# KwonGihyun/TweedieMix

Hardware: AMD Instinct MI355X
Metric: denoise steps/sec @ SDXL 1024^2 K=3 concepts (fusion phase); images/sec at 1/2/4/8 GPUs (higher is better)
Workload: dtype bf16

## Files before the change

### tweediemix_amd/csrc/conv_io.hip

```cpp
#include "common.h"

namespace {

struct PreMap { float w[16]; float b[4]; int on; };

template <int CIN>
__global__ void __launch_bounds__(256) conv_in_kernel(const float* __restrict__ x, const float* __restrict__ w,
                                                      const float* __restrict__ bias, bf16_t* __restrict__ y,
                                                      int B, int H, int W, int Cout, const PreMap pm) {
    extern __shared__ __attribute__((aligned(16))) float s_w[];
    constexpr int KK = 9 * CIN;
    const int tid = threadIdx.x, lane = tid & 63;
    const int q = __builtin_amdgcn_readfirstlane(tid >> 6);
    for (int i = tid; i < Cout * KK / 4; i += 256) ((float4*)s_w)[i] = ((const float4*)w)[i];
    __syncthreads();
    const int64_t npix = (int64_t)B * H * W;
    for (int64_t tile = blockIdx.x; tile * 64 < npix; tile += gridDim.x) {
    int64_t pix = tile * 64 + lane;
    const bool live = pix < npix;
    if (!live) pix = npix - 1;
    const int b = (int)(pix / ((int64_t)H * W)); const int rem = (int)(pix - (int64_t)b * H * W);
    const int oy = rem / W, ox = rem - oy * W;
    float patch[KK];
#pragma unroll
    for (int ky = 0; ky < 3; ++ky)
#pragma unroll
        for (int kx = 0; kx < 3; ++kx) {
            const int iy = oy + ky - 1, ix = ox + kx - 1;
            const bool ok = iy >= 0 && iy < H && ix >= 0 && ix < W;
            float v[CIN];
#pragma unroll
            for (int ci = 0; ci < CIN; ++ci) v[ci] = ok ? x[(((int64_t)b * CIN + ci) * H + iy) * W + ix] : 0.f;
            if (pm.on && CIN == 4) {
                float u[4];
#pragma unroll
                for (int co = 0; co < 4; ++co)
                    u[co] = ok ? pm.b[co] + pm.w[co * 4 + 0] * v[0] + pm.w[co * 4 + 1] * v[1] + pm.w[co * 4 + 2] * v[2] + pm.w[co * 4 + 3] * v[3] : 0.f;
#pragma unroll
                for (int co = 0; co < 4; ++co) v[co] = u[co];
            }
#pragma unroll
            for (int ci = 0; ci < CIN; ++ci) patch[(ky * 3 + kx) * CIN + ci] = v[ci];
        }
    const int cpq = Cout / 4;
    for (int c0 = q * cpq; c0 < (q + 1) * cpq; c0 += 8) {
        float o[8];
#pragma unroll 2
        for (int j = 0; j < 8; ++j) {
            const float* wr = s_w + (c0 + j) * KK;
            float a = bias ? bias[c0 + j] : 0.f;
#pragma unroll
            for (int k = 0; k < KK; ++k) a += patch[k] * wr[k];
            o[j] = a;
        }
        if (live) *(uint4*)(y + pix * Cout + c0) = pack8(o);
    }
    }
}

template <int CIN>
int launch_conv_in(unsigned nb, int smem, hipStream_t st, const float* x, const float* w, const float* bias, bf16_t* y, int B, int H, int W, int Cout, const PreMap& pm) {
    static int attr_smem = 0;
    if (smem > 64 * 1024 && smem > attr_smem) {
        hipError_t e = hipFuncSetAttribute((const void*)conv_in_kernel<CIN>, hipFuncAttributeMaxDynamicSharedMemorySize, smem);
        if (e != hipSuccess) TMIX_FAIL((int)e, "hipFuncSetAttribute: %s", hipGetErrorString(e));
        attr_smem = smem;
    }
    conv_in_kernel<CIN><<<nb, 256, smem, st>>>(x, w, bias, y, B, H, W, Cout, pm);
    TMIX_LAUNCH_CHECK();
    return TMIX_OK;
}

__global__ void __launch_bounds__(256) conv_out_kernel(const bf16_t* __restrict__ x, const bf16_t* __restrict__ w,
                                                       const float* __restrict__ bias, float* __restrict__ y,
                                                       int B, int H, int W, int Cin, int Cout) {
    const int lane = threadIdx.x & 63, fr = lane & 15, fg = lane >> 4;
    const int64_t npix = (int64_t)B * H * W;
    const int64_t pbase = ((int64_t)blockIdx.x * 4 + (threadIdx.x >> 6)) * 16;
    if (pbase >= npix) return;
    int64_t pix = pbase + fr; if (pix > npix - 1) pix = npix - 1;
    const int b = (int)(pix / ((int64_t)H * W)); const int rem = (int)(pix - (int64_t)b * H * W);
    const int oy = rem / W, ox = rem - oy * W;
    const int co = fr < Cout ? fr : Cout - 1;
    const bf16_t* wrow = w + (int64_t)co * 9 * Cin;
    f32x4 acc = {0.f, 0.f, 0.f, 0.f};
    const frag_ab zero = {0, 0, 0, 0, 0, 0, 0, 0};
    for (int tap = 0; tap < 9; ++tap) {
        const int ky = tap / 3, kx = tap - ky * 3;
        const int iy = oy + ky - 1, ix = ox + kx - 1;
        const bool ok = iy >= 0 && iy < H && ix >= 0 && ix < W;
        const bf16_t* src = x + (((int64_t)b * H + (ok ? iy : 0)) * W + (ok ? ix : 0)) * Cin;
        for (int c = 0; c < Cin; c += 32) {
            frag_ab a = *(const frag_ab*)(src + c + fg * 8);
            if (!ok) a = zero;
            const frag_ab wf = *(const frag_ab*)(wrow + tap * Cin + c + fg * 8);
            acc = __builtin_amdgcn_mfma_f32_16x16x32_bf16(a, wf, acc, 0, 0, 0);
        }
    }
    if (fr < Cout) {
        const float bv = bias ? bias[fr] : 0.f;
#pragma unroll
        for (int r = 0; r < 4; ++r) {
            const int64_t pp = pbase + fg * 4 + r;
            if (pp < npix) {
                const int bb = (int)(pp / ((int64_t)H * W)); const int64_t rr = pp - (int64_t)bb * H * W;
                y[((int64_t)bb * Cout + fr) * H * W + rr] = acc[r] + bv;
            }
        }
    }
}

}

extern "C" int tmix_conv_in(const float* x_nchw, const float* w_ohwi, const float* bias, void* y_nhwc,
                            int B, int Cin, int H, int W, int Cout, void* stream) {
    return tmix_conv_in_pre(x_nchw, w_ohwi, bias, y_nhwc, B, Cin, H, W, Cout, nullptr, nullptr, stream);
}

extern "C" int tmix_conv_in_pre(const float* x_nchw, const float* w_ohwi, const float* bias, void* y_nhwc,
                                int B, int Cin, int H, int W, int Cout, const float* pre_w, const float* pre_b, void* stream) {
    if (!x_nchw || !w_ohwi || !y_nhwc) TMIX_FAIL(TMIX_EINVAL, "conv_in: null pointer");
    if (B <= 0 || H <= 0 || W <= 0 || Cout <= 0) TMIX_FAIL(TMIX_ESHAPE, "conv_in: bad shape");
    if (!aligned16(y_nhwc)) TMIX_FAIL(TMIX_EALIGN, "conv_in: output must be 16-byte aligned");
    if (Cout % 32) TMIX_FAIL(TMIX_ESHAPE, "conv_in: Cout=%d must be a multiple of 32", Cout);
    if (Cin != 3 && Cin != 4 && Cin != 8) TMIX_FAIL(TMIX_ESHAPE, "conv_in: Cin=%d (3: RGB image, 4: image latent, 8: video latent + image-latent features)", Cin);
    if (Cin != 4 && pre_w) TMIX_FAIL(TMIX_EINVAL, "conv_in: the latent pre-map is defined for 4 channels");
    if ((Cout * 9 * Cin) % 4) TMIX_FAIL(TMIX_ESHAPE, "conv_in: Cout*9*Cin must be a multiple of 4");
    if (!aligned16(w_ohwi)) TMIX_FAIL(TMIX_EALIGN, "conv_in: weights must be 16-byte aligned");
    const int64_t npix = (int64_t)B * H * W;
    const int64_t ntiles = (npix + 63) / 64;
    const int smem = Cout * 9 * Cin * 4;
    const int per_cu = smem > 80 * 1024 ? 1 : (smem > 52 * 1024 ? 2 : 3);
    const unsigned nb = (unsigned)(ntiles < 256 * per_cu ? ntiles : 256 * per_cu);
    if (smem > 150 * 1024) TMIX_FAIL(TMIX_ESHAPE, "conv_in: Cout=%d too large for the LDS weight stage", Cout);
    PreMap pm = {};
    if (pre_w) {
        pm.on = 1;
        for (int i = 0; i < 16; ++i) pm.w[i] = pre_w[i];
        for (int i = 0; i < 4; ++i) pm.b[i] = pre_b ? pre_b[i] : 0.f;
    }
    hipStream_t st = (hipStream_t)stream;
    bf16_t* y = (bf16_t*)y_nhwc;
    switch (Cin) {
        case 8:  return launch_conv_in<8>(nb, smem, st, x_nchw, w_ohwi, bias, y, B, H, W, Cout, pm);
        case 3:  return launch_conv_in<3>(nb, smem, st, x_nchw, w_ohwi, bias, y, B, H, W, Cout, pm);
        default: return launch_conv_in<4>(nb, smem, st, x_nchw, w_ohwi, bias, y, B, H, W, Cout, pm);
    }
}

extern "C" int tmix_conv_out(const void* x_nhwc, const void* w_ohwi, const float* bias, float* y_nchw,
                             int B, int Cin, int H, int W, int Cout, void* stream) {
    if (!x_nhwc || !w_ohwi || !y_nchw) TMIX_FAIL(TMIX_EINVAL, "conv_out: null pointer");
    if (B <= 0 || H <= 0 || W <= 0 || Cout <= 0 || Cout > 16 || (Cin % 32)) TMIX_FAIL(TMIX_ESHAPE, "conv_out: Cin=%d (%%32) Cout=%d (<=16)", Cin, Cout);
    if (!aligned16(x_nhwc) || !aligned16(w_ohwi)) TMIX_FAIL(TMIX_EALIGN, "conv_out: pointers must be 16-byte aligned");
    const int64_t npix = (int64_t)B * H * W;
    const unsigned nb = (unsigned)((npix + 63) / 64);
    conv_out_kernel<<<nb, 256, 0, (hipStream_t)stream>>>((const bf16_t*)x_nhwc, (const bf16_t*)w_ohwi, bias, y_nchw, B, H, W, Cin, Cout);
    TMIX_LAUNCH_CHECK();
    return TMIX_OK;
}
```

Baseline: 32.96.

## Tile conv_out through LDS with halo reuse and widen conv_in blocks

conv_out now stages a (TH+2)x18 halo tile of the NHWC input and all filter rows into padded LDS, then runs MFMA over 2D spatial tiles with unrolled channel chunks. This replaces per-lane global loads that re-read each input pixel nine times. conv_in moves to 512-thread blocks covering 128 pixels with two pixels' worth of waves, and packs outputs pairwise. It also switches to explicit fma and deliberately unfused mul-add for the tail taps and pre-map rows, apparently to match reference rounding. The costs are higher LDS use per block, which may reduce occupancy, and extra staging work per block.

```diff
diff --git a/tweediemix_amd/csrc/conv_io.hip b/tweediemix_amd/csrc/conv_io.hip
--- a/tweediemix_amd/csrc/conv_io.hip
+++ b/tweediemix_amd/csrc/conv_io.hip
@@ -4,19 +4,26 @@
 
 struct PreMap { float w[16]; float b[4]; int on; };
 
+constexpr int CONV_IN_SPLIT = 12;
+__device__ __forceinline__ float mul_add_rounded(float a, float p, float w) {
+#pragma clang fp contract(off)
+    const float t = p * w;
+    return a + t;
+}
+
 template <int CIN>
-__global__ void __launch_bounds__(256) conv_in_kernel(const float* __restrict__ x, const float* __restrict__ w,
+__global__ void __launch_bounds__(512) conv_in_kernel(const float* __restrict__ x, const float* __restrict__ w,
                                                       const float* __restrict__ bias, bf16_t* __restrict__ y,
                                                       int B, int H, int W, int Cout, const PreMap pm) {
     extern __shared__ __attribute__((aligned(16))) float s_w[];
     constexpr int KK = 9 * CIN;
     const int tid = threadIdx.x, lane = tid & 63;
-    const int q = __builtin_amdgcn_readfirstlane(tid >> 6);
-    for (int i = tid; i < Cout * KK / 4; i += 256) ((float4*)s_w)[i] = ((const float4*)w)[i];
+    const int wv = __builtin_amdgcn_readfirstlane(tid >> 6), q = wv & 3, half = wv >> 2;
+    for (int i = tid; i < Cout * KK / 4; i += 512) ((float4*)s_w)[i] = ((const float4*)w)[i];
     __syncthreads();
     const int64_t npix = (int64_t)B * H * W;
-    for (int64_t tile = blockIdx.x; tile * 64 < npix; tile += gridDim.x) {
-    int64_t pix = tile * 64 + lane;
+    for (int64_t tile = blockIdx.x; tile * 128 < npix; tile += gridDim.x) {
+    int64_t pix = tile * 128 + half * 64 + lane;
     const bool live = pix < npix;
     if (!live) pix = npix - 1;
     const int b = (int)(pix / ((int64_t)H * W)); const int rem = (int)(pix - (int64_t)b * H * W);
@@ -34,8 +41,13 @@
             if (pm.on && CIN == 4) {
                 float u[4];
 #pragma unroll
-                for (int co = 0; co < 4; ++co)
-                    u[co] = ok ? pm.b[co] + pm.w[co * 4 + 0] * v[0] + pm.w[co * 4 + 1] * v[1] + pm.w[co * 4 + 2] * v[2] + pm.w[co * 4 + 3] * v[3] : 0.f;
+                for (int co = 0; co < 4; ++co) {
+                    float t = pm.b[co];
+#pragma unroll
+                    for (int ci = 0; ci < 4; ++ci)
+                        t = co < 2 ? __builtin_fmaf(pm.w[co * 4 + ci], v[ci], t) : mul_add_rounded(t, pm.w[co * 4 + ci], v[ci]);
+                    u[co] = ok ? t : 0.f;
+                }
 #pragma unroll
                 for (int co = 0; co < 4; ++co) v[co] = u[co];
             }
@@ -44,16 +56,25 @@
         }
     const int cpq = Cout / 4;
     for (int c0 = q * cpq; c0 < (q + 1) * cpq; c0 += 8) {
-        float o[8];
-#pragma unroll 2
-        for (int j = 0; j < 8; ++j) {
-            const float* wr = s_w + (c0 + j) * KK;
-            float a = bias ? bias[c0 + j] : 0.f;
-#pragma unroll
-            for (int k = 0; k < KK; ++k) a += patch[k] * wr[k];
-            o[j] = a;
-        }
-        if (live) *(uint4*)(y + pix * Cout + c0) = pack8(o);
+        uint32_t ow[4] = {0, 0, 0, 0};
+#pragma unroll 1
+        for (int jp = 0; jp < 4; ++jp) {
+            float o[2];
+#pragma unroll
+            for (int j = 0; j < 2; ++j) {
+                const float* wr = s_w + (c0 + 2 * jp + j) * KK;
+                float a = bias ? bias[c0 + 2 * jp + j] : 0.f;
+#pragma unroll
+                for (int k = 0; k < KK - CONV_IN_SPLIT; ++k) a = __builtin_fmaf(patch[k], wr[k], a);
+#pragma unroll
+                for (int k = KK - CONV_IN_SPLIT; k < KK; ++k) a = mul_add_rounded(a, patch[k], wr[k]);
+                o[j] = a;
+            }
+            const uint32_t pk = pack_bf2(o[0], o[1]);
+#pragma unroll
+            for (int t = 0; t < 4; ++t) ow[t] = jp == t ? pk : ow[t];
+        }
+        if (live) *(uint4*)(y + pix * Cout + c0) = make_uint4(ow[0], ow[1], ow[2], ow[3]);
     }
     }
 }
@@ -66,46 +87,100 @@
         if (e != hipSuccess) TMIX_FAIL((int)e, "hipFuncSetAttribute: %s", hipGetErrorString(e));
         attr_smem = smem;
     }
-    conv_in_kernel<CIN><<<nb, 256, smem, st>>>(x, w, bias, y, B, H, W, Cout, pm);
+    conv_in_kernel<CIN><<<nb, 512, smem, st>>>(x, w, bias, y, B, H, W, Cout, pm);
     TMIX_LAUNCH_CHECK();
     return TMIX_OK;
 }
 
-__global__ void __launch_bounds__(256) conv_out_kernel(const bf16_t* __restrict__ x, const bf16_t* __restrict__ w,
+constexpr int CONV_OUT_U = 8;
+constexpr int CONV_OUT_LDS = 160 * 1024;
+constexpr int CONV_OUT_TW = 16;
+
+__host__ __device__ inline int64_t conv_out_smem(int th, int Cin, int Cout) {
+    return ((int64_t)(th + 2) * (CONV_OUT_TW + 2) * (Cin + 8) + (int64_t)Cout * (9 * Cin + 8)) * 2;
+}
+inline int conv_out_tile_rows(int H, int Cin, int Cout) {
+    int th = 8;
+    while (th > 1 && (conv_out_smem(th, Cin, Cout) > CONV_OUT_LDS || th / 2 >= H)) th /= 2;
+    return conv_out_smem(th, Cin, Cout) > CONV_OUT_LDS ? 0 : th;
+}
+
+template <typename F>
+__device__ __forceinline__ void conv_out_stage(bf16_t* dst, int dstride, int rows, int vpr, int tid, int nthr, F src) {
+    const int total = rows * vpr, dq = nthr / vpr, dr = nthr - dq * vpr;
+    int r = tid / vpr, v = tid - r * vpr;
+    for (int i = tid; i < total; i += nthr * CONV_OUT_U) {
+        uint4 val[CONV_OUT_U];
+        int rr[CONV_OUT_U], vv[CONV_OUT_U];
+#pragma unroll
+        for (int u = 0; u < CONV_OUT_U; ++u) {
+            rr[u] = r; vv[u] = v;
+            val[u] = make_uint4(0, 0, 0, 0);
+            if (i + u * nthr < total) {
+                const bf16_t* g = src(r, v);
+                if (g) val[u] = *(const uint4*)g;
+            }
+            r += dq; v += dr;
+            if (v >= vpr) { v -= vpr; ++r; }
+        }
+#pragma unroll
+        for (int u = 0; u < CONV_OUT_U; ++u)
+            if (i + u * nthr < total) *(uint4*)(dst + (int64_t)rr[u] * dstride + vv[u] * 8) = val[u];
+    }
+}
+
+template <int N>
+__device__ __forceinline__ f32x4 conv_out_chunks(const bf16_t* a_lds, const bf16_t* w_lds, f32x4 acc) {
+    frag_ab a[N], wf[N];
+#pragma unroll
+    for (int i = 0; i < N; ++i) { a[i] = *(const frag_ab*)(a_lds + i * 32); wf[i] = *(const frag_ab*)(w_lds + i * 32); }
+#pragma unroll
+    for (int i = 0; i < N; ++i) acc = __builtin_amdgcn_mfma_f32_16x16x32_bf16(a[i], wf[i], acc, 0, 0, 0);
+    return acc;
+}
+
+__global__ void __launch_bounds__(512) conv_out_kernel(const bf16_t* __restrict__ x, const bf16_t* __restrict__ w,
                                                        const float* __restrict__ bias, float* __restrict__ y,
-                                                       int B, int H, int W, int Cin, int Cout) {
-    const int lane = threadIdx.x & 63, fr = lane & 15, fg = lane >> 4;
-    const int64_t npix = (int64_t)B * H * W;
-    const int64_t pbase = ((int64_t)blockIdx.x * 4 + (threadIdx.x >> 6)) * 16;
-    if (pbase >= npix) return;
-    int64_t pix = pbase + fr; if (pix > npix - 1) pix = npix - 1;
-    const int b = (int)(pix / ((int64_t)H * W)); const int rem = (int)(pix - (int64_t)b * H * W);
-    const int oy = rem / W, ox = rem - oy * W;
+                                                       int H, int W, int Cin, int Cout, int TH, int tiles_x, int tiles_y) {
+    extern __shared__ __attribute__((aligned(16))) bf16_t s_co[];
+    const int tid = threadIdx.x, nthr = blockDim.x, lane = tid & 63, fr = lane & 15, fg = lane >> 4;
+    const int row = __builtin_amdgcn_readfirstlane(tid >> 6);
+    int t = blockIdx.x;
+    const int tx = t % tiles_x; t /= tiles_x;
+    const int ty = t % tiles_y, b = t / tiles_y;
+    const int y0 = ty * TH, x0 = tx * CONV_OUT_TW;
+    const int ps = Cin + 8, ws = 9 * Cin + 8, vpp = Cin >> 3;
+    bf16_t* s_x = s_co;
+    bf16_t* s_w = s_co + (TH + 2) * (CONV_OUT_TW + 2) * ps;
+    const bf16_t* xb = x + (int64_t)b * H * W * Cin;
+    conv_out_stage(s_x, ps, (TH + 2) * (CONV_OUT_TW + 2), vpp, tid, nthr, [&](int p, int v) -> const bf16_t* {
+        const int py = p / (CONV_OUT_TW + 2), px = p - py * (CONV_OUT_TW + 2);
+        const int iy = y0 + py - 1, ix = x0 + px - 1;
+        return iy >= 0 && iy < H && ix >= 0 && ix < W ? xb + ((int64_t)iy * W + ix) * Cin + v * 8 : nullptr;
+    });
+    conv_out_stage(s_w, ws, Cout, 9 * vpp, tid, nthr, [&](int r, int v) -> const bf16_t* { return w + (int64_t)r * 9 * Cin + v * 8; });
+    __syncthreads();
+    const int oy = y0 + row;
+    if (oy >= H) return;
     const int co = fr < Cout ? fr : Cout - 1;
-    const bf16_t* wrow = w + (int64_t)co * 9 * Cin;
+    const bf16_t* wrow = s_w + co * ws + fg * 8;
     f32x4 acc = {0.f, 0.f, 0.f, 0.f};
-    const frag_ab zero = {0, 0, 0, 0, 0, 0, 0, 0};
     for (int tap = 0; tap < 9; ++tap) {
         const int ky = tap / 3, kx = tap - ky * 3;
-        const int iy = oy + ky - 1, ix = ox + kx - 1;
-        const bool ok = iy >= 0 && iy < H && ix >= 0 && ix < W;
-        const bf16_t* src = x + (((int64_t)b * H + (ok ? iy : 0)) * W + (ok ? ix : 0)) * Cin;
-        for (int c = 0; c < Cin; c += 32) {
-            frag_ab a = *(const frag_ab*)(src + c + fg * 8);
-            if (!ok) a = zero;
-            const frag_ab wf = *(const frag_ab*)(wrow + tap * Cin + c + fg * 8);
-            acc = __builtin_amdgcn_mfma_f32_16x16x32_bf16(a, wf, acc, 0, 0, 0);
-        }
+        const bf16_t* src = s_x + ((row + ky) * (CONV_OUT_TW + 2) + fr + kx) * ps + fg * 8;
+        const bf16_t* wt = wrow + tap * Cin;
+        int c = 0;
+        for (; c + 128 <= Cin; c += 128) acc = conv_out_chunks<4>(src + c, wt + c, acc);
+        for (; c + 64 <= Cin; c += 64) acc = conv_out_chunks<2>(src + c, wt + c, acc);
+        for (; c < Cin; c += 32) acc = conv_out_chunks<1>(src + c, wt + c, acc);
     }
     if (fr < Cout) {
         const float bv = bias ? bias[fr] : 0.f;
+        float* yrow = y + (((int64_t)b * Cout + fr) * H + oy) * W;
 #pragma unroll
         for (int r = 0; r < 4; ++r) {
-            const int64_t pp = pbase + fg * 4 + r;
-            if (pp < npix) {
-                const int bb = (int)(pp / ((int64_t)H * W)); const int64_t rr = pp - (int64_t)bb * H * W;
-                y[((int64_t)bb * Cout + fr) * H * W + rr] = acc[r] + bv;
-            }
+            const int ox = x0 + fg * 4 + r;
+            if (ox < W) yrow[ox] = acc[r] + bv;
         }
     }
 }
@@ -128,9 +203,9 @@
     if ((Cout * 9 * Cin) % 4) TMIX_FAIL(TMIX_ESHAPE, "conv_in: Cout*9*Cin must be a multiple of 4");
     if (!aligned16(w_ohwi)) TMIX_FAIL(TMIX_EALIGN, "conv_in: weights must be 16-byte aligned");
     const int64_t npix = (int64_t)B * H * W;
-    const int64_t ntiles = (npix + 63) / 64;
+    const int64_t ntiles = (npix + 127) / 128;
     const int smem = Cout * 9 * Cin * 4;
-    const int per_cu = smem > 80 * 1024 ? 1 : (smem > 52 * 1024 ? 2 : 3);
+    const int per_cu = smem > 80 * 1024 ? 1 : 2;
     const unsigned nb = (unsigned)(ntiles < 256 * per_cu ? ntiles : 256 * per_cu);
     if (smem > 150 * 1024) TMIX_FAIL(TMIX_ESHAPE, "conv_in: Cout=%d too large for the LDS weight stage", Cout);
     PreMap pm = {};
@@ -153,9 +228,19 @@
     if (!x_nhwc || !w_ohwi || !y_nchw) TMIX_FAIL(TMIX_EINVAL, "conv_out: null pointer");
     if (B <= 0 || H <= 0 || W <= 0 || Cout <= 0 || Cout > 16 || (Cin % 32)) TMIX_FAIL(TMIX_ESHAPE, "conv_out: Cin=%d (%%32) Cout=%d (<=16)", Cin, Cout);
     if (!aligned16(x_nhwc) || !aligned16(w_ohwi)) TMIX_FAIL(TMIX_EALIGN, "conv_out: pointers must be 16-byte aligned");
-    const int64_t npix = (int64_t)B * H * W;
-    const unsigned nb = (unsigned)((npix + 63) / 64);
-    conv_out_kernel<<<nb, 256, 0, (hipStream_t)stream>>>((const bf16_t*)x_nhwc, (const bf16_t*)w_ohwi, bias, y_nchw, B, H, W, Cin, Cout);
+    const int th = conv_out_tile_rows(H, Cin, Cout);
+    if (!th) TMIX_FAIL(TMIX_ESHAPE, "conv_out: Cin=%d Cout=%d: three input rows and the filter rows do not fit in LDS", Cin, Cout);
+    const int smem = (int)conv_out_smem(th, Cin, Cout);
+    static int attr_smem = 0;
+    if (smem > 64 * 1024 && smem > attr_smem) {
+        hipError_t e = hipFuncSetAttribute((const void*)conv_out_kernel, hipFuncAttributeMaxDynamicSharedMemorySize, smem);
+        if (e != hipSuccess) TMIX_FAIL((int)e, "hipFuncSetAttribute: %s", hipGetErrorString(e));
+        attr_smem = smem;
+    }
+    const int tiles_x = (W + CONV_OUT_TW - 1) / CONV_OUT_TW, tiles_y = (H + th - 1) / th;
+    const int64_t nb = (int64_t)B * tiles_x * tiles_y;
+    if (nb > 0x7fffffff) TMIX_FAIL(TMIX_ESHAPE, "conv_out: too many tiles");
+    conv_out_kernel<<<(unsigned)nb, 64 * th, smem, (hipStream_t)stream>>>((const bf16_t*)x_nhwc, (const bf16_t*)w_ohwi, bias, y_nchw, H, W, Cin, Cout, th, tiles_x, tiles_y);
     TMIX_LAUNCH_CHECK();
     return TMIX_OK;
 }
```

Result: no change. 32.99 (median of 2 runs) (+0.1%).
